# WilliamFlinchbaugh/Deep-RL-Battlespace

Measured on AMD Instinct MI355X. Metric: agent-steps/sec, higher is better.
Workload: dtype f64/i16

## Files before the change

deep-rl-battlespace_amd/csrc/bsx_kernels.hip:

```cpp

#include <array>
#include <mutex>
#include <unordered_map>

#include "bsx_config.h"
#include "bsx_args.h"
#include "bsx_state.h"
#include "bsx_rng.h"
#include "bsx_geometry.h"
#include "bsx_instinct.h"
#include "bsx_step_kernel.h"
#define BSX_INST_PER_CALL
#define BSX_INST_MULTI_TICK
#define BSX_INST_ROLLOUT
#include "bsx_step_split.h"
#define BSX_INST_SPLIT_MANY
#define BSX_INST_SPLIT
#define BSX_INST_SPLIT_CONT
#ifdef BSX_VARIANT
#define BSX_INST_KW
#else
#define BSX_INST_KW extern
#endif
#include "bsx_step_instances.h"
using namespace bsxk;

namespace {

struct ResetArgs {
    StatePtrs st; int64_t E; int n; const uint8_t* mask; const int32_t* spawn; uint64_t seed; uint64_t nonce;
    int64_t env_offset; float* obs; int observe_only;
};

__global__ __launch_bounds__(TPB) void bsx_reset_kernel(const ResetArgs p) {
    const int n = p.n, A = 2 * n, G = group_width(n), EPB = TPB / G;
    const int tid = threadIdx.x, a = tid & (G - 1), gl = tid & ~(G - 1);
    const int64_t e = int64_t(blockIdx.x) * EPB + (tid / G);
    const bool env_ok = e < p.E, valid = env_ok && a < A;
    const size_t g = valid ? size_t(e) * A + a : 0;
    __shared__ volatile int s_x[TPB], s_y[TPB], s_hp[TPB];

    EnvU er = {};
    uint32_t games = 0;
    int x = 0, y = 0, hp = 0;
    double dir = 0.0;
    bool frac = false;
    if (env_ok) {
        const uint2 dw = p.st.envd[e];
        er = unpack_env(p.st.envc[e], dw.x);
        games = dw.y;
    }
    if (valid) {
        const uint2 pw = p.st.plane[g];
        unpack_plane(pw, x, y, hp, dir);
        frac = (pw.y & PLANE_FRAC) != 0u;
        if (frac) dir = p.st.pdirf[g];
    }
    const bool doit = env_ok && !p.observe_only && (!p.mask || p.mask[e]);
    if (p.spawn) {
        if (doit) {
            const int32_t* s = p.spawn + size_t(e) * (4 + 3 * A);
            er.brx = s[0]; er.bry = s[1]; er.bbx = s[2]; er.bby = s[3];
            if (valid) { x = s[4 + 3 * a]; y = s[5 + 3 * a]; dir = double(s[6 + 3 * a]); }
        }
    } else if (!p.observe_only) {
        const int64_t genv = p.env_offset + (env_ok ? e : p.E - 1);
        const int ac = a < A ? a : A - 1;
        const SpawnDraw sd = spawn_from_words(draw4(p.seed, genv, STREAM_RESET, uint32_t(p.nonce), uint32_t(ac)), ac, n);
        const int lane0 = (tid & 63) & ~(G - 1);
        const int rbx = __shfl(sd.bx, lane0), rby = __shfl(sd.by, lane0), bbx = __shfl(sd.bx, lane0 + n), bby = __shfl(sd.by, lane0 + n);
        if (doit) {
            er.brx = rbx; er.bry = rby; er.bbx = bbx; er.bby = bby;
            if (valid) { x = sd.x; y = sd.y; dir = double(sd.dir); }
        }
    }
    if (doit) {
        er.bhp_r = er.bhp_b = 5 * n;
        er.tick = 0; er.done = 0; er.winner = BSX_WINNER_NONE;
        hp = PLANE_HP; frac = false;
        if (valid) p.st.plane[g] = pack_plane(x, y, hp, dir, false);
        if (valid && a == 0) { p.st.envc[e] = pack_envc(er); p.st.envd[e] = make_uint2(pack_envd(er), games); }
    }
    if (!p.observe_only) {
        const int lane = tid & 63;
        const int64_t wb = int64_t(blockIdx.x) * (TPB / 64) + (tid >> 6);
        const unsigned long long resetting = __ballot(doit);
        if (resetting != 0ull && wb < wave_blocks(p.E, n)) {
            uint2* const pool = p.st.bent + size_t(wb) * POOL_CAP;
            const int pc = int(p.st.bcnt[wb]);
            int wpos = 0;
            for (int base = 0; base < pc; base += 64) {
                const int w = base + lane;
                const uint2 en = pool[w < pc ? w : 0];
                const bool stay = w < pc && ((resetting >> (en.x >> ENT_OWNER_SHIFT)) & 1ull) == 0ull;
                const unsigned long long kb = __ballot(stay);
                const int ps = wpos + __popcll(kb & ((1ull << lane) - 1ull));
                if (stay) pool[ps] = en;
                wpos += __popcll(kb);
            }
            if (lane == 0) p.st.bcnt[wb] = uint32_t(wpos);
        }
    }
    s_x[tid] = x; s_y[tid] = y; s_hp[tid] = valid ? hp : 0;
    __syncthreads();
    if (valid && p.obs) {
        const int team = a < n ? 0 : 1;
        write_obs<0>(p.obs + g * size_t(3 * n + 2), n, hp > 0, x, y, dir, a,
                     team == 0 ? er.bbx : er.brx, team == 0 ? er.bby : er.bry, gl, s_x, s_y, s_hp);
    }
}

__global__ void bsx_mark_done_kernel(uint2* envd, int64_t E) {
    const int64_t e = int64_t(blockIdx.x) * blockDim.x + threadIdx.x;
    if (e < E) envd[e] = make_uint2(1u << 27, 0u);
}

struct ExportArgs { StatePtrs st; int64_t E; int n; BsxExport out; int tie_tick; };

__global__ __launch_bounds__(TPB) void bsx_export_kernel(const ExportArgs p) {
    const int A = 2 * p.n;
    const size_t EA = size_t(p.E) * A;
    const size_t g = size_t(blockIdx.x) * TPB + threadIdx.x;
    if (g >= EA) return;
    const int64_t e = int64_t(g / A);
    const int a = int(g % A);
    const uint2 pw = p.st.plane[g];
    int x, y, hp;
    double dir;
    unpack_plane(pw, x, y, hp, dir);
    if (pw.y & PLANE_FRAC) dir = p.st.pdirf[g];
    const BsxExport& o = p.out;
    if (o.px) o.px[g] = x;
    if (o.py) o.py[g] = y;
    if (o.pdir) o.pdir[g] = dir;
    if (o.php) o.php[g] = hp;
    if (o.palive) o.palive[g] = hp > 0;
    const uint2 dw = p.st.envd[e];
    const EnvU ev = unpack_env(p.st.envc[e], dw.x);
    const int ptick = ev.tick - ((ev.done && ev.winner == BSX_WINNER_TIE && ev.tick >= p.tie_tick) ? 1 : 0);
    for (int k = 0; k < K; ++k) {
        const size_t i = g * K + k;
        if (o.bl_live) o.bl_live[i] = 0;
        if (o.bl_x) o.bl_x[i] = 0;
        if (o.bl_y) o.bl_y[i] = 0;
        if (o.bl_dir) o.bl_dir[i] = 0.0;
    }
    const int G = group_width(p.n), EPB = 64 / G;
    const int64_t wb = e / EPB;
    const uint32_t me = uint32_t(int(e % EPB) * G + a);
    const uint2* const pool = p.st.bent + size_t(wb) * POOL_CAP;
    const int cnt = int(p.st.bcnt[wb]);
    for (int j2 = 0; j2 < cnt; ++j2) {
        const uint32_t w = pool[j2].x;
        const int age = bullet_age(w);
        if ((w >> ENT_OWNER_SHIFT) != me || age == int(TOMBSTONE_AGE)) continue;
        int slot = (ptick - age + 1) % K;
        if (slot < 0) slot += K;
        const size_t i = g * K + slot;
        if (o.bl_live) o.bl_live[i] = 1;
        if (o.bl_x) o.bl_x[i] = bullet_x(w);
        if (o.bl_y) o.bl_y[i] = bullet_y(w);
        if (o.bl_dir) o.bl_dir[i] = p.st.bdir[size_t(slot) * EA + g];
    }
    if (a == 0) {
        if (o.base_xy) { o.base_xy[4 * e] = ev.brx; o.base_xy[4 * e + 1] = ev.bry; o.base_xy[4 * e + 2] = ev.bbx; o.base_xy[4 * e + 3] = ev.bby; }
        if (o.bhp) { o.bhp[2 * e] = ev.bhp_r; o.bhp[2 * e + 1] = ev.bhp_b; }
        if (o.tick) o.tick[e] = ev.tick;
        if (o.env_done) o.env_done[e] = ev.done;
        if (o.winner) o.winner[e] = ev.winner;
        if (o.counters) {
            const int* c4 = p.st.cnt + 4 * e;
            o.counters[4 * e] = c4[0]; o.counters[4 * e + 1] = c4[1]; o.counters[4 * e + 2] = c4[2]; o.counters[4 * e + 3] = c4[3];
        }
    }
}

struct InstinctArgs {
    const float* obs; void* actions; const double* rnd; int64_t E; int n; int team; int out_kind; int continuous;
    uint64_t seed; uint64_t seq; const uint64_t* seq_base; int64_t env_offset;
};

__global__ __launch_bounds__(TPB) void bsx_instinct_kernel(const InstinctArgs p) {
    const int A = 2 * p.n, D = 3 * p.n + 2;
    const size_t g = size_t(blockIdx.x) * TPB + threadIdx.x;
    if (g >= size_t(p.E) * A) return;
    const int a = int(g % A);
    const int tm = a < p.n ? 0 : 1;
    if (p.team != 2 && p.team != tm) return;
    const float* o = p.obs + g * D;
    double td, ta;
    const int act = instinct_choose([&](int k) { return o[k]; }, p.n, td, ta);
    if (!p.continuous) {
        if (p.out_kind == BSX_ACT_I32) static_cast<int32_t*>(p.actions)[g] = act;
        else static_cast<float4*>(p.actions)[g] = one_hot_scores(act);
        return;
    }
    double r0, n0, n1, n2;
    if (p.rnd) { r0 = p.rnd[4 * g]; n0 = p.rnd[4 * g + 1]; n1 = p.rnd[4 * g + 2]; n2 = p.rnd[4 * g + 3]; }
    else instinct_continuous_draws(p.seed, p.seq + (p.seq_base ? *p.seq_base : 0ull), uint64_t(p.env_offset) * uint64_t(A) + g, r0, n0, n1, n2);
    double* out = static_cast<double*>(p.actions) + 3 * g;
    instinct_continuous_action(td, ta, r0, n0, n1, n2, out[0], out[1], out[2]);
}

std::mutex g_family_mu;
std::unordered_map<const void*, int> g_family;
inline void family_forget(const void* state) {
    std::lock_guard<std::mutex> lk(g_family_mu);
    g_family.erase(state);
}
inline bool family_claim(const void* state, bool cont) {
    std::lock_guard<std::mutex> lk(g_family_mu);
    int& f = g_family[state];
    if (f == 0) f = cont ? 2 : 1;
    return f == (cont ? 2 : 1);
}
inline int grid_for(int64_t E, int n) {
    const int epb = TPB / group_width(n);
    return int((E + epb - 1) / epb);
}

inline bool narrow_offsets_ok(int64_t E, int n, uint32_t flags) {
    return !(flags & BSX_F_WIDE_OFFSETS) && uint64_t(E) * uint64_t(2 * n) * 200ull <= 0xFFFFFFFFull;
}
constexpr int64_t SPLIT_MAX_GAMES = 114688, SPLIT_MANY_MAX_GAMES = 65536, SPLIT_CONT_MAX_GAMES = 81920;
constexpr int64_t SPLIT_DRAW_MAX_GAMES = 98304;
constexpr int64_t SPLIT_MANY_FORM2_FROM = 32768;
template <bool CONT, bool MULTI>
inline bool split_applies(int n, const StepArgs& a, int64_t bound) {
    if (n != 1 || (a.flags & BSX_F_ONE_WAVE)) return false;
    if (CONT) return !MULTI && bound <= SPLIT_CONT_MAX_GAMES;
    return bound <= (MULTI ? SPLIT_MANY_MAX_GAMES : SPLIT_MAX_GAMES);
}

using StepKernel = void (*)(BSX_STEP_KERNEL_PARAMS);

template <class F>
StepKernel by_team_and_offsets(int n, bool off32, F f) {
    const auto w = [&](auto N) { return off32 ? f(N, std::true_type{}) : f(N, std::false_type{}); };
    switch (n) {
        case 1: return w(std::integral_constant<int, 1>{});
        case 2: return w(std::integral_constant<int, 2>{});
        case 3: return w(std::integral_constant<int, 3>{});
        case 4: return w(std::integral_constant<int, 4>{});
        default: return w(std::integral_constant<int, 0>{});
    }
}

template <bool CONT, bool MULTI, bool ACTOR, bool LG>
int launch_for_n(const StepArgs& a, int64_t bound, void* stream) {
    const int n = a.n;
    const bool two_wave = !ACTOR && split_applies<CONT, MULTI>(n, a, bound);
    const StepKernel k = by_team_and_offsets(n, narrow_offsets_ok(a.E, n, a.flags), [&](auto N_, auto OFF32_) -> StepKernel {
        constexpr int N = decltype(N_)::value;
        constexpr bool OFF32 = decltype(OFF32_)::value;
        if constexpr (ACTOR) {
            if constexpr (N == 0) return nullptr;
            else return bsx_step_kernel<N, CONT, true, true, false, OFF32>;
        } else {
            if constexpr (N == 1 && !(CONT && MULTI)) {
                if (two_wave) {
                    if constexpr (MULTI)
                        return bound > SPLIT_MANY_FORM2_FROM ? bsx_step_split_kernel<LG, OFF32, 2>
                                                             : bsx_step_split_kernel<LG, OFF32, 1>;
                    else if constexpr (CONT)
                        return bsx_step_split_kernel<false, OFF32, 0, true, true>;
                    else
                        return bound <= SPLIT_DRAW_MAX_GAMES ? bsx_step_split_kernel<LG, OFF32, 0, false, true>
                                                             : bsx_step_split_kernel<LG, OFF32, 0>;
                }
            }
            return bsx_step_kernel<N, CONT, MULTI, false, LG, OFF32>;
        }
    });
    const StepGeometry geo = step_geometry(ACTOR ? FORM_ROLLOUT : (two_wave ? FORM_TWO_WAVE : FORM_ONE_WAVE), bound, n);
    const dim3 grid(unsigned(geo.groups));
    const dim3 block(SPB * geo.waves);
    hipLaunchKernelGGL(k, grid, block, 0, static_cast<hipStream_t>(stream),
                       bound, a.st.envc, a.st.envd, a.st.plane, a.actions, a.st.bent, a.st.bcnt, a.action_kind, a);
    return int(hipGetLastError());
}

StepArgs step_args(void* state, int64_t E, int n, int T, float* rew, uint8_t* done, uint8_t* env_done, uint8_t* winner,
                   uint8_t* env_done_t, const BsxRewards* cfg, uint32_t flags, uint64_t seed, int64_t env_offset) {
    StepArgs a{};
    a.st = state_ptrs(state, E, n);
    a.E = E; a.n = n; a.T = T;
    a.rew = rew; a.done = done; a.env_done = env_done; a.winner = winner; a.env_done_t = env_done_t;
    a.cfg = *cfg; a.flags = flags; a.seed = seed; a.env_offset = env_offset; a.tie_tick = tie_tick_const(n);
    a.scripted_team = -1;
    return a;
}

struct StepCall { int64_t first = 0, count = -1; int T = 0; int store_all = 0; uint8_t* env_done_t = nullptr; };

template <bool CONT>
int step(const StepCall& c, void* state, int64_t E, int n, const void* actions, int action_kind, const double* u, float* obs, float* rew,
         uint8_t* done, uint8_t* env_done, uint8_t* winner, const BsxRewards* cfg, uint32_t flags, uint64_t seed, int64_t env_offset,
         void* stream) {
    const int T = c.T;
    const int64_t first = c.first, count = c.count < 0 ? E - first : c.count;
    if (T < 0 || T > BSX_MAX_T || first < 0 || count <= 0 || first > E - count || (first & 255) || ((first || count != E) && T != 0))
        return BSX_E_ARG;
    if (!obs || !rew || !done || !cfg || (!actions && (T || !(flags & BSX_F_EMPTY_CALL)))) return BSX_E_ARG;
    if (const int rc = check_games(state, E, n)) return rc;
    if (!aligned(obs, 4) || !aligned(rew, 4) || (u && !aligned(u, 8))) return BSX_E_ALIGN;
    if (!CONT && action_kind == BSX_ACT_LOGITS_F32 && !aligned(actions, 16)) return BSX_E_ALIGN;
    if (!CONT && action_kind != BSX_ACT_I32 && action_kind != BSX_ACT_LOGITS_F32) return BSX_E_ARG;
    if (CONT && action_kind != BSX_ACT_F32 && action_kind != BSX_ACT_F64 && action_kind != BSX_ACT_F32X4) return BSX_E_ARG;
    if (CONT && action_kind == BSX_ACT_F32X4 && !aligned(actions, 16)) return BSX_E_ALIGN;
    if (!family_claim(state, CONT)) return BSX_E_FAMILY;
    StepArgs a = step_args(state, E, n, T, rew, done, env_done, winner, c.env_done_t, cfg, flags, seed, env_offset);
    a.actions = actions; a.action_kind = action_kind; a.u = u; a.obs = obs;
    if (!actions) { a.actions = state; a.action_kind = -1; }
    const int64_t EA = E * 2 * n;
    a.act_tb = EA * (CONT ? (action_kind == BSX_ACT_F32 ? 12 : (action_kind == BSX_ACT_F64 ? 24 : 16)) : (action_kind == BSX_ACT_I32 ? 4 : 16));
    a.u_ts = EA;
    a.obs_ts = c.store_all ? EA * (3 * n + 2) : 0; a.rew_ts = c.store_all ? EA : 0; a.done_ts = c.store_all ? EA : 0;
    if (first) {
        const int64_t fa = first * 2 * n;
        const int64_t fb = first / (64 / group_width(n));
        a.st.envc += first; a.st.envd += first; a.st.cnt += 4 * first; a.st.plane += fa; a.st.pdirf += fa;
        a.st.bcnt += fb; a.st.bent += fb * POOL_CAP; a.st.bdir += fa; a.st.bd += fa;
        if (actions) a.actions = static_cast<const char*>(actions) + fa * (a.act_tb / EA);
        if (u) a.u += fa;
        a.obs += fa * (3 * n + 2); a.rew += fa; a.done += fa;
        if (env_done) a.env_done += first;
        if (winner) a.winner += first;
        a.env_offset += first;
    }
    const bool lg = !CONT && action_kind == BSX_ACT_LOGITS_F32;
    if (T == 0) return lg ? launch_for_n<CONT, false, false, !CONT>(a, count, stream) : launch_for_n<CONT, false, false, false>(a, count, stream);
    return lg ? launch_for_n<CONT, true, false, !CONT>(a, count, stream) : launch_for_n<CONT, true, false, false>(a, count, stream);
}

template <bool CONT>
int rollout(void* state, int64_t E, int n, int T, const float* weights, int precision, int scripted_team, uint64_t scripted_seed, float* obs,
            float* scores, float* rew, uint8_t* done, uint8_t* env_done, uint8_t* winner, uint8_t* env_done_t, const BsxRewards* cfg,
            uint32_t flags, const BsxActorNoise* noise, uint64_t actor_seed, uint64_t seq, const uint64_t* seq_base, uint64_t seed,
            int64_t env_offset, void* stream, bool gauss = false, const BsxGaussianHead* head = nullptr) {
    if (T < 1 || T > BSX_MAX_T || !weights || !obs || !scores || !rew || !done || !cfg || (flags & BSX_F_EMPTY_CALL) ||
        (precision != BSX_ACTOR_F32 && precision != BSX_ACTOR_BF16X3 && precision != BSX_ACTOR_BF16X6) || scripted_team < -1 || scripted_team > 1)
        return BSX_E_ARG;
    if (gauss && (!head || !head->log_std)) return BSX_E_ARG;
    if (const int rc = check_games(state, E, n, 256, ROLLOUT_MAX_N)) return rc;
    if (!aligned(weights, 16) || !aligned(scores, 16) || !aligned(obs, 4) || !aligned(rew, 4)) return BSX_E_ALIGN;
    BsxActorNoise nz = {};
    if (noise) nz = *noise;
    if (gauss) {
        if (nz.gaussian_std > 0.f || nz.ou_scale > 0.f || nz.sample_mode != 0 || nz.u_inject || nz.logp) return BSX_E_ARG;
        if (!aligned(head->log_std, 4) || (head->logp && !aligned(head->logp, 4))) return BSX_E_ALIGN;
    }
    if (nz.ou_scale > 0.f && (!nz.ou_state || !aligned(nz.ou_state, 16))) return nz.ou_state ? BSX_E_ALIGN : BSX_E_ARG;
    if (nz.z_inject || nz.u_inject) return BSX_E_ARG;
    if (nz.sample_mode != 0 && (nz.sample_mode != 1 || !(nz.temperature > 0.f) || CONT)) return BSX_E_ARG;
    if ((nz.logp && !aligned(nz.logp, 4)) || (nz.value_weights && !aligned(nz.value_weights, 16))) return BSX_E_ALIGN;
    if (nz.value_weights && (n != 1 || !nz.value || !aligned(nz.value, 4))) return BSX_E_ARG;
    if (!family_claim(state, CONT)) return BSX_E_FAMILY;
    const int64_t EA = E * 2 * n, D = 3 * n + 2;
    StepArgs a = step_args(state, E, n, T, rew, done, env_done, winner, env_done_t, cfg, flags, seed, env_offset);
    a.action_kind = CONT ? BSX_ACT_F32X4 : BSX_ACT_LOGITS_F32;
    a.obs = obs + EA * D; a.obs_ts = EA * D; a.rew_ts = EA; a.done_ts = EA;
    a.aw = weights; a.aprec = precision; a.scripted_team = scripted_team; a.obs0 = obs; a.scores = scores; a.scores_ts = EA * 4; a.nz = nz;
    a.aseed = actor_seed; a.aseq = seq; a.aseq_base = seq_base; a.iseed = scripted_seed;
    if (gauss) a.gh = *head;
    return launch_for_n<CONT, true, true, false>(a, E, stream);
}

const std::array<double2, 361>& heading_table() {
    static const std::array<double2, 361> lut = [] {
        std::array<double2, 361> t;
        const double st = 215 * 0.1;
        for (int d = 0; d <= 360; ++d) {
            const double ang = -(double(d) * DEG2RAD);
            t[d].x = st * cos(ang);
            t[d].y = st * sin(ang);
        }
        return t;
    }();
    return lut;
}

}

extern "C" {

int bsx_abi_version(void) { return BSX_ABI_VERSION; }

int bsx_build_flags(void) { return BUILD_FLAGS; }

int bsx_stream_synchronize(void* stream) { return int(hipStreamSynchronize(static_cast<hipStream_t>(stream))); }

int bsx_host_device_pointer(void* host, void** device) {
    if (!host || !device) return BSX_E_ARG;
    return int(hipHostGetDevicePointer(device, host, 0));
}

int bsx_tie_tick(int n) { return tie_tick_const(n); }

int bsx_state_bytes(int64_t E, int n, size_t* bytes) {
    if (const int rc = check_games(bytes, E, n, 1)) return rc;
    *bytes = make_layout(E, n).total;
    return 0;
}

int bsx_state_init(void* state, int64_t E, int n, void* stream) {
    if (const int rc = check_games(state, E, n)) return rc;
    const Layout L = make_layout(E, n);
    family_forget(state);
    hipStream_t s = static_cast<hipStream_t>(stream);
    hipError_t err = hipMemsetAsync(state, 0, L.total, s);
    if (err != hipSuccess) return int(err);
    const std::array<double2, 361>& lut = heading_table();
    err = hipMemcpyAsync(static_cast<char*>(state) + L.lut, lut.data(), sizeof(double2) * lut.size(), hipMemcpyHostToDevice, s);
    if (err != hipSuccess) return int(err);
    hipLaunchKernelGGL(bsx_mark_done_kernel, dim3(unsigned((E + TPB - 1) / TPB)), dim3(TPB), 0, s,
                       reinterpret_cast<uint2*>(static_cast<char*>(state) + L.envd), E);
    return int(hipGetLastError());
}

int bsx_state_release(void* state) {
    if (!state) return BSX_E_ARG;
    family_forget(state);
    return 0;
}

int bsx_reset(void* state, int64_t E, int n, const uint8_t* reset_mask, const int32_t* spawn, uint64_t seed,
              uint64_t nonce, int64_t env_offset, float* obs, void* stream) {
    if (const int rc = check_games(state, E, n)) return rc;
    if ((spawn && !aligned(spawn, 4)) || (obs && !aligned(obs, 4))) return BSX_E_ALIGN;
    if (!reset_mask) family_forget(state);
    ResetArgs a{state_ptrs(state, E, n), E, n, reset_mask, spawn, seed, nonce, env_offset, obs, 0};
    hipLaunchKernelGGL(bsx_reset_kernel, dim3(grid_for(E, n)), dim3(TPB), 0, static_cast<hipStream_t>(stream), a);
    return int(hipGetLastError());
}

int bsx_step_discrete(void* state, int64_t E, int n, const void* actions, int action_kind, const double* u, float* obs,
                      float* rew, uint8_t* done, uint8_t* env_done, uint8_t* winner, const BsxRewards* cfg,
                      uint32_t flags, uint64_t seed, int64_t env_offset, void* stream) {
    return step<false>({}, state, E, n, actions, action_kind, u, obs, rew, done, env_done, winner, cfg, flags, seed, env_offset, stream);
}

int bsx_step_continuous(void* state, int64_t E, int n, const void* actions, int action_kind, const double* u,
                        float* obs, float* rew, uint8_t* done, uint8_t* env_done, uint8_t* winner,
                        const BsxRewards* cfg, uint32_t flags, uint64_t seed, int64_t env_offset, void* stream) {
    return step<true>({}, state, E, n, actions, action_kind, u, obs, rew, done, env_done, winner, cfg, flags, seed, env_offset, stream);
}

int bsx_step_discrete_range(void* state, int64_t E, int n, int64_t first, int64_t count, const void* actions, int action_kind, const double* u,
                            float* obs, float* rew, uint8_t* done, uint8_t* env_done, uint8_t* winner, const BsxRewards* cfg,
                            uint32_t flags, uint64_t seed, int64_t env_offset, void* stream) {
    return step<false>({first, count}, state, E, n, actions, action_kind, u, obs, rew, done, env_done, winner, cfg, flags, seed, env_offset, stream);
}

int bsx_step_continuous_range(void* state, int64_t E, int n, int64_t first, int64_t count, const void* actions, int action_kind, const double* u,
                              float* obs, float* rew, uint8_t* done, uint8_t* env_done, uint8_t* winner, const BsxRewards* cfg,
                              uint32_t flags, uint64_t seed, int64_t env_offset, void* stream) {
    return step<true>({first, count}, state, E, n, actions, action_kind, u, obs, rew, done, env_done, winner, cfg, flags, seed, env_offset, stream);
}

int bsx_step_many_discrete(void* state, int64_t E, int n, int T, const void* actions, int action_kind, const double* u,
                           float* obs, float* rew, uint8_t* done, uint8_t* env_done, uint8_t* winner, uint8_t* env_done_t, const BsxRewards* cfg,
                           uint32_t flags, int store_all, uint64_t seed, int64_t env_offset, void* stream) {
    return T < 1 ? BSX_E_ARG : step<false>({0, -1, T, store_all, env_done_t}, state, E, n, actions, action_kind, u, obs, rew, done, env_done,
                                           winner, cfg, flags, seed, env_offset, stream);
}

int bsx_step_many_continuous(void* state, int64_t E, int n, int T, const void* actions, int action_kind, const double* u,
                             float* obs, float* rew, uint8_t* done, uint8_t* env_done, uint8_t* winner, uint8_t* env_done_t, const BsxRewards* cfg,
                             uint32_t flags, int store_all, uint64_t seed, int64_t env_offset, void* stream) {
    return T < 1 ? BSX_E_ARG : step<true>({0, -1, T, store_all, env_done_t}, state, E, n, actions, action_kind, u, obs, rew, done, env_done,
                                          winner, cfg, flags, seed, env_offset, stream);
}

int bsx_rollout_discrete(void* state, int64_t E, int n, int T, const float* weights, int precision, int scripted_team, float* obs, float* scores, float* rew,
                         uint8_t* done, uint8_t* env_done, uint8_t* winner, uint8_t* env_done_t, const BsxRewards* cfg, uint32_t flags,
                         const BsxActorNoise* noise, uint64_t actor_seed, uint64_t seq, const uint64_t* seq_base, uint64_t seed,
                         int64_t env_offset, void* stream) {
    return rollout<false>(state, E, n, T, weights, precision, scripted_team, 0, obs, scores, rew, done, env_done, winner, env_done_t, cfg, flags,
                          noise, actor_seed, seq, seq_base, seed, env_offset, stream);
}

int bsx_rollout_continuous(void* state, int64_t E, int n, int T, const float* weights, int precision, int scripted_team, uint64_t scripted_seed, float* obs, float* scores, float* rew,
                           uint8_t* done, uint8_t* env_done, uint8_t* winner, uint8_t* env_done_t, const BsxRewards* cfg, uint32_t flags,
                           const BsxActorNoise* noise, uint64_t actor_seed, uint64_t seq, const uint64_t* seq_base, uint64_t seed,
                           int64_t env_offset, void* stream) {
    return rollout<true>(state, E, n, T, weights, precision, scripted_team, scripted_seed, obs, scores, rew, done, env_done, winner, env_done_t, cfg, flags,
                         noise, actor_seed, seq, seq_base, seed, env_offset, stream);
}

int bsx_rollout_continuous_gaussian(void* state, int64_t E, int n, int T, const float* weights, int precision, int scripted_team,
                                    uint64_t scripted_seed, float* obs, float* scores, float* rew,
                                    uint8_t* done, uint8_t* env_done, uint8_t* winner, uint8_t* env_done_t, const BsxRewards* cfg,
                                    uint32_t flags, const BsxActorNoise* noise, const BsxGaussianHead* head, uint64_t actor_seed,
                                    uint64_t seq, const uint64_t* seq_base, uint64_t seed, int64_t env_offset, void* stream) {
    return rollout<true>(state, E, n, T, weights, precision, scripted_team, scripted_seed, obs, scores, rew, done, env_done, winner, env_done_t, cfg, flags,
                         noise, actor_seed, seq, seq_base, seed, env_offset, stream, true, head);
}

__global__ void bsx_selftest_atan2_kernel(int R, unsigned long long* out) {
    const int W = 2 * R + 1;
    const long long total = (long long)W * W;
    unsigned long long bad = 0, seen = 0;
    for (long long i = (long long)blockIdx.x * blockDim.x + threadIdx.x; i < total; i += (long long)gridDim.x * blockDim.x) {
        const int iy = int(i / W) - R, ix = int(i % W) - R;
        const double lib = atan2(double(iy), double(ix));
        const double one = atan2_pixels(iy, ix);
        const int ys[3] = {iy, ix, -iy}, xs[3] = {ix, iy, ix};
        double three[3];
        atan2_pixels_n<3>(ys, xs, three);
        const bool ok = __double_as_longlong(one) == __double_as_longlong(lib) && __double_as_longlong(three[0]) == __double_as_longlong(lib) &&
                        __double_as_longlong(three[1]) == __double_as_longlong(atan2(double(ix), double(iy))) &&
                        __double_as_longlong(three[2]) == __double_as_longlong(atan2(double(-iy), double(ix)));
        bad += ok ? 0ull : 1ull;
        seen += 1ull;
    }
    atomicAdd(&out[0], bad); atomicAdd(&out[1], seen);
}
int bsx_selftest_atan2(int R, uint64_t* out, void* stream) {
    if (!out || R < 0 || R > 4096) return BSX_E_ARG;
    hipStream_t st = static_cast<hipStream_t>(stream);
    hipError_t err = hipMemsetAsync(out, 0, 2 * sizeof(uint64_t), st);
    if (err != hipSuccess) return int(err);
    bsx_selftest_atan2_kernel<<<1024, 256, 0, st>>>(R, reinterpret_cast<unsigned long long*>(out));
    return int(hipGetLastError());
}

int bsx_observe(void* state, int64_t E, int n, float* obs, void* stream) {
    if (!obs) return BSX_E_ARG;
    if (const int rc = check_games(state, E, n)) return rc;
    if (!aligned(obs, 4)) return BSX_E_ALIGN;
    ResetArgs a{state_ptrs(state, E, n), E, n, nullptr, nullptr, 0, 0, 0, obs, 1};
    hipLaunchKernelGGL(bsx_reset_kernel, dim3(grid_for(E, n)), dim3(TPB), 0, static_cast<hipStream_t>(stream), a);
    return int(hipGetLastError());
}

int bsx_export_state(const void* state, int64_t E, int n, const BsxExport* out, void* stream) {
    if (!out) return BSX_E_ARG;
    if (const int rc = check_games(state, E, n)) return rc;
    ExportArgs a{state_ptrs(const_cast<void*>(state), E, n), E, n, *out, bsx_tie_tick(n)};
    const size_t EA = size_t(E) * 2 * n;
    hipLaunchKernelGGL(bsx_export_kernel, dim3(unsigned((EA + TPB - 1) / TPB)), dim3(TPB), 0,
                       static_cast<hipStream_t>(stream), a);
    return int(hipGetLastError());
}

int bsx_instinct_discrete(const float* obs, void* actions, int out_kind, int64_t E, int n, int team, void* stream) {
    if (!actions || team < 0 || team > 2 || (out_kind != BSX_ACT_I32 && out_kind != BSX_ACT_LOGITS_F32)) return BSX_E_ARG;
    if (const int rc = check_games(obs, E, n, 4)) return rc;
    if (!aligned(actions, out_kind == BSX_ACT_I32 ? 4 : 16)) return BSX_E_ALIGN;
    InstinctArgs a{obs, actions, nullptr, E, n, team, out_kind, 0, 0, 0, nullptr, 0};
    const size_t EA = size_t(E) * 2 * n;
    hipLaunchKernelGGL(bsx_instinct_kernel, dim3(unsigned((EA + TPB - 1) / TPB)), dim3(TPB), 0, static_cast<hipStream_t>(stream), a);
    return int(hipGetLastError());
}

int bsx_instinct_continuous_shard(const float* obs, double* actions, const double* rnd, int64_t E, int n, int team,
                                  uint64_t seed, uint64_t seq, const uint64_t* seq_base, int64_t env_offset, void* stream) {
    if (!actions || team < 0 || team > 2 || env_offset < 0) return BSX_E_ARG;
    if (const int rc = check_games(obs, E, n, 4)) return rc;
    if (!aligned(actions, 8) || (rnd && !aligned(rnd, 8))) return BSX_E_ALIGN;
    InstinctArgs a{obs, actions, rnd, E, n, team, 0, 1, seed, seq, seq_base, env_offset};
    const size_t EA = size_t(E) * 2 * n;
    hipLaunchKernelGGL(bsx_instinct_kernel, dim3(unsigned((EA + TPB - 1) / TPB)), dim3(TPB), 0, static_cast<hipStream_t>(stream), a);
    return int(hipGetLastError());
}

int bsx_instinct_continuous(const float* obs, double* actions, const double* rnd, int64_t E, int n, int team,
                            uint64_t seed, uint64_t seq, const uint64_t* seq_base, void* stream) {
    return bsx_instinct_continuous_shard(obs, actions, rnd, E, n, team, seed, seq, seq_base, 0, stream);
}

}
```

deep-rl-battlespace_amd/csrc/bsx_step_kernel.h:

```cpp
#pragma once

namespace bsxk {

__device__ inline int argmax4(float a, float b, float c, float d) {
    int am = 0;
    float best = a;
    const float v[3] = {b, c, d};
#pragma unroll
    for (int i = 0; i < 3; ++i)
        if (!(best != best) && (v[i] > best || v[i] != v[i])) { am = i + 1; best = v[i]; }
    return am;
}

struct StepArgs {
    StatePtrs st;
    int64_t E; int n;
    const void* actions; int action_kind;
    const double* u;
    float* obs; float* rew; uint8_t* done; uint8_t* env_done; uint8_t* winner;
    uint8_t* env_done_t;
    BsxRewards cfg;
    uint32_t flags; uint64_t seed; int64_t env_offset; int tie_tick;
    int T; int64_t act_tb , u_ts, obs_ts, rew_ts, done_ts ;
    const float* aw; int aprec; int scripted_team ; const float* obs0; float* scores; int64_t scores_ts; BsxActorNoise nz; uint64_t aseed, aseq; const uint64_t* aseq_base;
    uint64_t iseed;
    BsxGaussianHead gh;
};

#define BSX_STEP_KERNEL_PARAMS                                                                                                           \
    const int64_t E_, const uint2* const envc_, const uint2* const envd_, const uint2* const plane_, const void* const act_,               \
        const uint2* const bent_, const uint32_t* const bcnt_, const int kind_, const bsxk::StepArgs p_

template <int N>
__device__ inline void write_obs(float* __restrict__ out, int n, bool alive, int x, int y, double dir, int a,
                                 int ebx, int eby, int gl, const volatile int* s_x, const volatile int* s_y,
                                 const volatile int* s_hp) {
    const int D = 3 * n + 2;
    if (!alive || (DIAG & 1u)) {
        for (int i = 0; i < D; ++i) out[i] = -1.0f;
        return;
    }
    out[0] = obs_dist(x, y, ebx, eby);
    out[1] = obs_angle(x, y, dir, ebx, eby);
    const int eb = gl + (a < n ? n : 0);
    for (int j = 0; j < n; ++j) {
        if (s_hp[eb + j] > 0) {
            const int qx = s_x[eb + j], qy = s_y[eb + j];
            out[2 + 3 * j] = 1.0f;
            out[3 + 3 * j] = obs_dist(x, y, qx, qy);
            out[4 + 3 * j] = obs_angle(x, y, dir, qx, qy);
        } else {
            out[2 + 3 * j] = -1.0f; out[3 + 3 * j] = -1.0f; out[4 + 3 * j] = -1.0f;
        }
    }
}

enum Mode : int { M_INERT = 0, M_TIE = 1, M_PHYS = 2, M_RESET = 3 };

constexpr int tie_tick_const(int n) {
    const double max_time = double(10 + n * 2);
    double t = 0.0;
    int k = 0;
    do { t += 0.1; ++k; } while (!(t >= max_time));
    return k;
}
static_assert(tie_tick_const(1) == 121 && tie_tick_const(2) == 141 && tie_tick_const(3) == 161 && tie_tick_const(4) == 181 &&
              tie_tick_const(5) == 200, "time-limit tick");
static_assert(tie_tick_const(BSX_MAX_N) < 512, "the game clock fits the 9 bits of the game record");

template <class T> __device__ inline T* elem(T* base, uint32_t i) {
    typedef typename std::conditional<std::is_const<T>::value, const char, char>::type byte_t;
    return reinterpret_cast<T*>(reinterpret_cast<byte_t*>(base) + uint32_t(i * uint32_t(sizeof(T))));
}
template <class T> __device__ inline T* elem(T* base, size_t i) { return base + i; }
__device__ inline void end_of_tick() {
    __builtin_amdgcn_fence(__ATOMIC_RELEASE, "wavefront");
    __builtin_amdgcn_wave_barrier();
    __builtin_amdgcn_fence(__ATOMIC_ACQUIRE, "wavefront");
}
template <int N, bool CONT, bool MULTI, bool ACTOR = false, bool LG = false, bool OFF32 = false>
__global__ __launch_bounds__(SPB * (ACTOR ? group_width(N > 0 ? N : 1) / 2 : WPB)) __attribute__((amdgpu_waves_per_eu((ACTOR && N > 1) ? 2 : ((!ACTOR && MULTI && N == 2) ? 4 : 1))))
void bsx_step_kernel(BSX_STEP_KERNEL_PARAMS) {
    const StepArgs& p = p_;
    const unsigned stamp_row = blockIdx.x; (void)stamp_row;
    STAMP(8);
    typedef typename std::conditional<OFF32, uint32_t, size_t>::type ix_t;
    typedef typename std::conditional<OFF32, int32_t, int64_t>::type ixs_t;
    constexpr bool NT_STATE = !MULTI && N >= 2;
    constexpr int WAVES = ACTOR ? group_width(N > 0 ? N : 1) / 2 : WPB;
    const int n = (N > 0) ? N : p.n;
    const int A = 2 * n;
    const int G = group_width(n);
    const int EPB = SPB / G;
    const int wave = (WAVES > 1) ? int(threadIdx.x >> 6) : 0;
    const int tid = (WAVES > 1) ? int(threadIdx.x & 63) : int(threadIdx.x);
    const ixs_t wblk = (WAVES > 1) ? ixs_t(blockIdx.x) * WAVES + wave : ixs_t(blockIdx.x);
    const int a = tid & (G - 1);
    const ixs_t e = wblk * EPB + (tid / G);
    const bool env_ok = e < ixs_t(E_);
    const bool valid = env_ok && a < A;
    const ix_t EA = ix_t((MULTI || ACTOR) ? E_ : p.E) * ix_t(A);
    const ixs_t ec = env_ok ? e : ixs_t(E_ - 1);
    const ix_t g = ix_t(ec) * A + (a < A ? a : A - 1);
    constexpr int MANY = -1; constexpr bool DRAW = false;
#include "bsx_step_lds.inl"

    const bool has_act = kind_ >= 0;
    struct RawIn { int ai; float4 lg; float f0, f1, f2; double c0, c1, c2, uu; };
    auto load_inputs = [&](int t, RawIn& r) {
        const void* const at = MULTI ? static_cast<const void*>(static_cast<const char*>(act_) + int64_t(t) * p.act_tb) : act_;
        const double* const ut = (MULTI && p.u) ? p.u + int64_t(t) * p.u_ts : p.u;
        if (!CONT) {
            const char* const abase = static_cast<const char*>(at);
            if constexpr (LG) r.lg = *reinterpret_cast<const float4*>(elem(abase, has_act ? g * 16 : ix_t(0)));
            else r.ai = *reinterpret_cast<const int32_t*>(elem(abase, has_act ? g * 4 : ix_t(0)));
        } else if (has_act) {
            if (kind_ == BSX_ACT_F32) {
                const float* ap = static_cast<const float*>(at) + 3 * g;
                r.f0 = ap[0]; r.f1 = ap[1]; r.f2 = ap[2];
            } else if (kind_ == BSX_ACT_F32X4) {
                const float4 v = static_cast<const float4*>(at)[g];
                r.f0 = v.x; r.f1 = v.y; r.f2 = v.z;
            } else {
                const double* ap = static_cast<const double*>(at) + 3 * g;
                r.c0 = ap[0]; r.c1 = ap[1]; r.c2 = ap[2];
            }
        }
        __builtin_amdgcn_sched_barrier(0);
        if (ut) r.uu = ut[g];
    };
    int x = 0, y = 0, hp = 0;
    uint32_t games = 0;
    double dir = 0.0;
    EnvU er = {};
    const ix_t pool0 = ix_t(wblk) * ix_t(POOL_CAP);
    uint32_t pc = 0;
    uint2 pool_first = make_uint2(0u, 0u);
    RawIn rin = {}, rin_next = {};
    struct DecIn { int act; double a0, a1, a2, uu; };
    auto decode = [&](const RawIn& r) {
        DecIn d = {-1, 0.0, 0.0, 0.0, 0.0};
        if (has_act) {
            if (!CONT) {
                if constexpr (!LG) d.act = r.ai;
                else d.act = argmax4(r.lg.x, r.lg.y, r.lg.z, r.lg.w);
            } else if (kind_ == BSX_ACT_F32 || kind_ == BSX_ACT_F32X4) {
                d.a0 = double(r.f0); d.a1 = double(r.f1); d.a2 = double(r.f2);
            } else {
                d.a0 = r.c0; d.a1 = r.c1; d.a2 = r.c2;
            }
        }
        if (p.u) d.uu = r.uu;
        return d;
    };
    DecIn din_next = {-1, 0.0, 0.0, 0.0, 0.0};
    if (MULTI && !ACTOR) { load_inputs(0, rin_next); din_next = decode(rin_next); }
    if constexpr (ACTOR) {
        constexpr int D = 3 * N + 2;
        for (int i = int(threadIdx.x); i < 2 * N * bsx_actor::SMALL / 4; i += SPB * WAVES) {
            const int ag = i / (bsx_actor::SMALL / 4), j = i - ag * (bsx_actor::SMALL / 4);
            reinterpret_cast<float4*>(s_small)[i] =
                reinterpret_cast<const float4*>(p.aw + size_t(ag) * bsx_actor::blob_floats(D) + bsx_actor::off_small(D))[j];
        }
        if constexpr (N == 1) {
            if (p.nz.value_weights)
                for (int i = int(threadIdx.x); i < 2 * bsx_actor::SMALL / 4; i += SPB * WAVES) {
                    const int ag = i / (bsx_actor::SMALL / 4), j = i - ag * (bsx_actor::SMALL / 4);
                    reinterpret_cast<float4*>(s_small + 2 * bsx_actor::SMALL)[i] =
                        reinterpret_cast<const float4*>(p.nz.value_weights + size_t(ag) * bsx_actor::blob_floats(D) + bsx_actor::off_small(D))[j];
                }
        }
        const int64_t e_first = wblk * EPB;
        const int64_t nfl = min(int64_t(SPB), (E_ - e_first) * A) * D;
        if (G == A) {
            for (int i = tid; i < SPB * D; i += SPB) s_obs[i] = i < nfl ? p.obs0[size_t(e_first) * A * D + i] : -1.0f;
        } else {
            for (int k = 0; k < D; ++k) s_obs[tid * D + k] = valid ? p.obs0[g * D + k] : -1.0f;
        }
        __builtin_amdgcn_fence(__ATOMIC_RELEASE, "workgroup");
        if (WAVES > 1) __syncthreads(); else __builtin_amdgcn_wave_barrier();
        __builtin_amdgcn_fence(__ATOMIC_ACQUIRE, "workgroup");
    }

    for (int tk = 0; tk < (MULTI ? p.T : 1); ++tk) {
    ix_t gt = g, EAt = EA;
    uint64_t seed_t = p.seed;
    int64_t env_offset_t = p.env_offset;
    constexpr int TIE_C = tie_tick_const(N > 0 ? N : 1);
    int tie_tick = (N > 0) ? TIE_C : p.tie_tick;
    if (MULTI) {
        asm volatile("" : "+v"(gt));
        asm volatile("" : "+s"(EAt));
        asm volatile("" : "+s"(seed_t));
    }
    int tid_k = tid;
    if constexpr ((ACTOR && N > 1) || (MULTI && !ACTOR && N > 0 && ((OPAQUE_MULTI_MASK >> (((LG || CONT) ? 8 : 0) + N)) & 1))) asm volatile("" : "+v"(tid_k));
    typedef const StepArgs __attribute__((address_space(4))) StepArgsK;
    static_assert(alignof(StepArgs) == 8, "kernarg offset of StepArgs");
    const char __attribute__((address_space(4)))* ka = (const char __attribute__((address_space(4)))*)__builtin_amdgcn_kernarg_segment_ptr();
    if (MULTI) asm volatile("" : "+s"(ka));
    auto& p = [&]() -> decltype(auto) { if constexpr (MULTI) return (*reinterpret_cast<StepArgsK*>(ka + 64)); else return (p_); }();
    const int tid = tid_k, lane = tid, a = tid & (G - 1);
    const int gl = tid & ~(G - 1);
    const int team = (a < n) ? 0 : 1;
    const int eb = gl + (team == 0 ? n : 0);
    const double* const u_t = (MULTI && p.u) ? p.u + int64_t(tk) * p.u_ts : p.u;
    float* const obs_t = MULTI ? p.obs + int64_t(tk) * p.obs_ts : p.obs;
    float* const rew_t = MULTI ? p.rew + int64_t(tk) * p.rew_ts : p.rew;
    uint8_t* const done_t = MULTI ? p.done + int64_t(tk) * p.done_ts : p.done;
    STAMP(0);
    if (!MULTI || tk == 0) {
        const uint2 ecw = *elem(envc_, ix_t(ec));
        const uint2 edw = *elem(envd_, ix_t(ec));
        const uint2 prw = *elem(plane_, gt);
        double dirf = 0.0;
        pool_first = *elem(bent_, pool0 + ix_t(lane));
        if (!(DIAG & 2u)) pc = __builtin_amdgcn_readfirstlane(*elem(bcnt_, ix_t(wblk)));
        if constexpr (CONT) dirf = *elem(p.st.pdirf, gt);
        if (!MULTI) load_inputs(0, rin);
        if (!MULTI) {
            asm volatile("" : "+s"(seed_t), "+s"(env_offset_t));
            if (N == 0) asm volatile("" : "+s"(tie_tick));
        }
        unpack_plane(prw, x, y, hp, dir);
        if constexpr (CONT) dir = (prw.y & PLANE_FRAC) ? dirf : dir;
        er = unpack_env(ecw, edw.x);
        games = edw.y;
    } else {
        pool_first = *elem(bent_, pool0 + ix_t(lane));
    }
    const DecIn din = MULTI ? din_next : decode(rin);
    int act = din.act;
    double a0 = din.a0, a1 = din.a1, a2 = din.a2, uu_in = din.uu;
    constexpr bool R_BULLETS = true, R_MOVE = true, R_STAGE = true, R_GEOM = true, R_OUTCOME = true, R_ST_STATE = true, R_ST_OUT = true, R_POSE_LDS = false;
    constexpr int R_RDV_COUNTS = 0, R_GEOM_LDS = 0, R_PUB = 0, R_DRAW_LDS = 0;
    auto split_rendezvous = [] {};
#include "bsx_step_phase_actor.inl"
#include "bsx_step_phase_shot.inl"
#include "bsx_step_phase_move.inl"
#include "bsx_step_phase_geometry.inl"
#include "bsx_step_phase_bullets.inl"
#include "bsx_step_phase_outcome.inl"
#include "bsx_step_phase_stores.inl"
    STAMP(7);
    if (MULTI) {
        games += uint32_t(cnt_delta.x);
        end_of_tick();
        STAMP(9);
    }
    }
}

}
```

deep-rl-battlespace_amd/csrc/bsx_step_split.h:

```cpp
#pragma once

namespace bsxk {

template <bool LG, bool OFF32, int MANY = 0, bool CONT_ = false, bool DRAW = false>
__global__ __launch_bounds__(2 * SPB)
void bsx_step_split_kernel(BSX_STEP_KERNEL_PARAMS) {
    constexpr int N = 1;
    constexpr bool CONT = CONT_, MULTI = MANY != 0, ACTOR = false;
    static_assert(!CONT || (MANY == 0 && !LG), "continuous actions: the per-call form only");
    static_assert(!DRAW || MANY == 0, "the geometry wave's draw: the per-call form only");
    const StepArgs& p = p_;
    typedef typename std::conditional<OFF32, uint32_t, size_t>::type ix_t;
    typedef typename std::conditional<OFF32, int32_t, int64_t>::type ixs_t;
    constexpr bool NT_STATE = false;
    constexpr int WAVES = 1;
    const int n = 1, A = 2, G = 2, EPB = SPB / 2;
    const int wave = 0;
    const int role_wave = int(threadIdx.x >> 6);
    const unsigned stamp_row = blockIdx.x * 2u + unsigned(role_wave); (void)stamp_row;
    STAMP(8);
    STAMP_HWID();
    const int tid = int(threadIdx.x & 63);
    const ixs_t wblk = ixs_t(blockIdx.x);
    const int a = tid & (G - 1);
    const ixs_t e = wblk * EPB + (tid / G);
    const bool env_ok = e < ixs_t(E_);
    const bool valid = env_ok && a < A;
    const ix_t EA = ix_t(MULTI ? E_ : p.E) * ix_t(A);
    const ixs_t ec = env_ok ? e : ixs_t(E_ - 1);
    const ix_t g = ix_t(ec) * A + (a < A ? a : A - 1);
#include "bsx_step_lds.inl"
    auto split_rendezvous = [] {
        asm volatile("s_waitcnt lgkmcnt(0)\n\ts_barrier" ::: "memory");
    };
    const bool has_act = kind_ >= 0;
    struct RawIn { int ai; float4 lg; double uu; };
    struct DecIn { int act; double uu; };
    auto load_inputs = [&](int t, RawIn& r) {
        const char* const abase = static_cast<const char*>(act_) + (MULTI ? int64_t(t) * p.act_tb : int64_t(0));
        if constexpr (LG) r.lg = *reinterpret_cast<const float4*>(elem(abase, has_act ? g * 16 : ix_t(0)));
        else r.ai = *reinterpret_cast<const int32_t*>(elem(abase, has_act ? g * 4 : ix_t(0)));
        __builtin_amdgcn_sched_barrier(0);
        const double* const ut = (MULTI && p.u) ? p.u + int64_t(t) * p.u_ts : p.u;
        if (ut) r.uu = ut[g];
    };
    auto decode = [&](const RawIn& r) {
        DecIn d = {-1, 0.0};
        if (has_act) d.act = LG ? argmax4(r.lg.x, r.lg.y, r.lg.z, r.lg.w) : r.ai;
        if (p.u) d.uu = r.uu;
        return d;
    };
    const ix_t pool0 = ix_t(wblk) * ix_t(POOL_CAP);
    if constexpr (MANY != 0) {
        if (role_wave == 0) {
            __builtin_amdgcn_s_setprio(1);
            constexpr bool R_BULLETS = true, R_MOVE = true, R_STAGE = true, R_GEOM = false, R_OUTCOME = true, R_POSE_LDS = false;
            constexpr bool R_ST_STATE = MANY == 2, R_ST_OUT = false;
            constexpr int R_RDV_COUNTS = MANY == 2 ? 0 : 1, R_GEOM_LDS = 0, R_PUB = MANY == 2 ? 1 : 0, R_DRAW_LDS = 0;
            s_ov[tid] = 0ull;
#include "bsx_step_split_many_body.inl"
        } else if constexpr (MANY == 2) {
            constexpr bool R_BULLETS = false, R_GEOM = true, R_ST_STATE = false, R_ST_OUT = true;
            constexpr int R_GEOM_LDS = 0, R_PUB = 0;
#include "bsx_step_split_out_body.inl"
        } else {
            constexpr bool R_BULLETS = false, R_MOVE = true, R_STAGE = false, R_GEOM = true, R_OUTCOME = true, R_POSE_LDS = false;
            constexpr bool R_ST_STATE = true, R_ST_OUT = true;
            constexpr int R_RDV_COUNTS = 2, R_GEOM_LDS = 0, R_PUB = 0, R_DRAW_LDS = 0;
#include "bsx_step_split_many_body.inl"
        }
    } else {
        constexpr int R_PUB = 0;
        const int tk = 0;
        if (role_wave == 0) {
            __builtin_amdgcn_s_setprio(1);
            constexpr bool R_BULLETS = true, R_MOVE = true, R_STAGE = true, R_GEOM = false, R_OUTCOME = true, R_ST_STATE = true, R_ST_OUT = true;
            constexpr bool R_POSE_LDS = true;
            constexpr int R_RDV_COUNTS = 0, R_GEOM_LDS = 2, R_DRAW_LDS = DRAW ? 2 : 0;
            s_ov[tid] = 0ull;
#include "bsx_step_split_body.inl"
        } else {
#include "bsx_step_split_geom_body.inl"
        }
    }
}

}
```

Baseline: 24.07 billion.

## Shrink kernel header args, read StepArgs in place, and hoist state loads

Changes the kernel parameter list to pass E as 32-bit and packs n into the kind argument, so generic-N per-call kernels read StepArgs directly from the kernarg segment at a fixed offset instead of copying it. In the per-call path, the env/plane/bullet/count state loads and the action load are issued before the tick loop so their latency overlaps setup. Continuous action loads become one unified raw-triple load with the decode deferred. This adds a hard-coded kernarg offset, and E is truncated to int, which would overflow for very large environment counts.

```diff
diff --git a/deep-rl-battlespace_amd/csrc/bsx_kernels.hip b/deep-rl-battlespace_amd/csrc/bsx_kernels.hip
--- a/deep-rl-battlespace_amd/csrc/bsx_kernels.hip
+++ b/deep-rl-battlespace_amd/csrc/bsx_kernels.hip
@@ -275,8 +275,9 @@
     const StepGeometry geo = step_geometry(ACTOR ? FORM_ROLLOUT : (two_wave ? FORM_TWO_WAVE : FORM_ONE_WAVE), bound, n);
     const dim3 grid(unsigned(geo.groups));
     const dim3 block(SPB * geo.waves);
+    const int kind_n = (!MULTI && n > 4) ? ((n << 8) | (a.action_kind & 255)) : a.action_kind;
     hipLaunchKernelGGL(k, grid, block, 0, static_cast<hipStream_t>(stream),
-                       bound, a.st.envc, a.st.envd, a.st.plane, a.actions, a.st.bent, a.st.bcnt, a.action_kind, a);
+                       int(bound), kind_n, a.st.envc, a.st.envd, a.st.plane, a.actions, a.st.bent, a.st.bcnt, a);
     return int(hipGetLastError());
 }
 
diff --git a/deep-rl-battlespace_amd/csrc/bsx_step_kernel.h b/deep-rl-battlespace_amd/csrc/bsx_step_kernel.h
--- a/deep-rl-battlespace_amd/csrc/bsx_step_kernel.h
+++ b/deep-rl-battlespace_amd/csrc/bsx_step_kernel.h
@@ -28,8 +28,10 @@
 };
 
 #define BSX_STEP_KERNEL_PARAMS                                                                                                           \
-    const int64_t E_, const uint2* const envc_, const uint2* const envd_, const uint2* const plane_, const void* const act_,               \
-        const uint2* const bent_, const uint32_t* const bcnt_, const int kind_, const bsxk::StepArgs p_
+    const int E_, const int kind_n_, const uint2* const envc_, const uint2* const envd_, const uint2* const plane_,                          \
+        const void* const act_, const uint2* const bent_, const uint32_t* const bcnt_, const bsxk::StepArgs p_
+constexpr int STEP_ARGS_KERNARG_OFFSET = 56;
+static_assert(STEP_ARGS_KERNARG_OFFSET % alignof(StepArgs) == 0, "kernarg offset of StepArgs");
 
 template <int N>
 __device__ inline void write_obs(float* __restrict__ out, int n, bool alive, int x, int y, double dir, int a,
@@ -73,6 +75,23 @@
     return reinterpret_cast<T*>(reinterpret_cast<byte_t*>(base) + uint32_t(i * uint32_t(sizeof(T))));
 }
 template <class T> __device__ inline T* elem(T* base, size_t i) { return base + i; }
+struct RawTriple { uint3 lo, hi; };
+template <class IX> __device__ inline RawTriple load_triple(const void* act, IX g, int kind, bool has_act) {
+    const char* const abase = static_cast<const char*>(act);
+    const IX stride = kind == BSX_ACT_F32 ? IX(12) : (kind == BSX_ACT_F64 ? IX(24) : IX(16));
+    const IX at = has_act ? g * stride : IX(0);
+    RawTriple r;
+    r.lo = *reinterpret_cast<const uint3*>(elem(abase, at));
+    r.hi = *reinterpret_cast<const uint3*>(elem(abase, at + (kind == BSX_ACT_F64 ? IX(12) : IX(0))));
+    return r;
+}
+__device__ inline void decode_triple(const RawTriple& r, int kind, double& a0, double& a1, double& a2) {
+    if (kind == BSX_ACT_F64) {
+        a0 = __hiloint2double(int(r.lo.y), int(r.lo.x)); a1 = __hiloint2double(int(r.hi.x), int(r.lo.z)); a2 = __hiloint2double(int(r.hi.z), int(r.hi.y));
+    } else {
+        a0 = double(__uint_as_float(r.lo.x)); a1 = double(__uint_as_float(r.lo.y)); a2 = double(__uint_as_float(r.lo.z));
+    }
+}
 __device__ inline void end_of_tick() {
     __builtin_amdgcn_fence(__ATOMIC_RELEASE, "wavefront");
     __builtin_amdgcn_wave_barrier();
@@ -81,14 +100,20 @@
 template <int N, bool CONT, bool MULTI, bool ACTOR = false, bool LG = false, bool OFF32 = false>
 __global__ __launch_bounds__(SPB * (ACTOR ? group_width(N > 0 ? N : 1) / 2 : WPB)) __attribute__((amdgpu_waves_per_eu((ACTOR && N > 1) ? 2 : ((!ACTOR && MULTI && N == 2) ? 4 : 1))))
 void bsx_step_kernel(BSX_STEP_KERNEL_PARAMS) {
-    const StepArgs& p = p_;
+    typedef const StepArgs __attribute__((address_space(4))) StepArgsK;
+    constexpr bool ARGS_IN_PLACE = N == 0 && !MULTI;
+    auto& p = [&]() -> decltype(auto) {
+        if constexpr (ARGS_IN_PLACE) return (*reinterpret_cast<StepArgsK*>((const char __attribute__((address_space(4)))*)__builtin_amdgcn_kernarg_segment_ptr() + STEP_ARGS_KERNARG_OFFSET));
+        else return (p_);
+    }();
     const unsigned stamp_row = blockIdx.x; (void)stamp_row;
     STAMP(8);
     typedef typename std::conditional<OFF32, uint32_t, size_t>::type ix_t;
     typedef typename std::conditional<OFF32, int32_t, int64_t>::type ixs_t;
     constexpr bool NT_STATE = !MULTI && N >= 2;
     constexpr int WAVES = ACTOR ? group_width(N > 0 ? N : 1) / 2 : WPB;
-    const int n = (N > 0) ? N : p.n;
+    const int kind_ = ARGS_IN_PLACE ? int(int8_t(kind_n_)) : kind_n_;
+    const int n = (N > 0) ? N : (ARGS_IN_PLACE ? (kind_n_ >> 8) : p.n);
     const int A = 2 * n;
     const int G = group_width(n);
     const int EPB = SPB / G;
@@ -99,35 +124,29 @@
     const ixs_t e = wblk * EPB + (tid / G);
     const bool env_ok = e < ixs_t(E_);
     const bool valid = env_ok && a < A;
-    const ix_t EA = ix_t((MULTI || ACTOR) ? E_ : p.E) * ix_t(A);
     const ixs_t ec = env_ok ? e : ixs_t(E_ - 1);
     const ix_t g = ix_t(ec) * A + (a < A ? a : A - 1);
     constexpr int MANY = -1; constexpr bool DRAW = false;
 #include "bsx_step_lds.inl"
 
     const bool has_act = kind_ >= 0;
-    struct RawIn { int ai; float4 lg; float f0, f1, f2; double c0, c1, c2, uu; };
-    auto load_inputs = [&](int t, RawIn& r) {
+    struct RawIn { int ai; float4 lg; RawTriple tr; double uu; };
+    auto load_action = [&](int t, RawIn& r) {
         const void* const at = MULTI ? static_cast<const void*>(static_cast<const char*>(act_) + int64_t(t) * p.act_tb) : act_;
-        const double* const ut = (MULTI && p.u) ? p.u + int64_t(t) * p.u_ts : p.u;
         if (!CONT) {
             const char* const abase = static_cast<const char*>(at);
             if constexpr (LG) r.lg = *reinterpret_cast<const float4*>(elem(abase, has_act ? g * 16 : ix_t(0)));
             else r.ai = *reinterpret_cast<const int32_t*>(elem(abase, has_act ? g * 4 : ix_t(0)));
-        } else if (has_act) {
-            if (kind_ == BSX_ACT_F32) {
-                const float* ap = static_cast<const float*>(at) + 3 * g;
-                r.f0 = ap[0]; r.f1 = ap[1]; r.f2 = ap[2];
-            } else if (kind_ == BSX_ACT_F32X4) {
-                const float4 v = static_cast<const float4*>(at)[g];
-                r.f0 = v.x; r.f1 = v.y; r.f2 = v.z;
-            } else {
-                const double* ap = static_cast<const double*>(at) + 3 * g;
-                r.c0 = ap[0]; r.c1 = ap[1]; r.c2 = ap[2];
-            }
-        }
+        } else r.tr = load_triple(at, g, kind_, has_act);
+    };
+    auto load_u = [&](int t, RawIn& r) {
+        const double* const ut = (MULTI && p.u) ? p.u + int64_t(t) * p.u_ts : p.u;
+        if (ut) r.uu = ut[g];
+    };
+    auto load_inputs = [&](int t, RawIn& r) {
+        load_action(t, r);
         __builtin_amdgcn_sched_barrier(0);
-        if (ut) r.uu = ut[g];
+        load_u(t, r);
     };
     int x = 0, y = 0, hp = 0;
     uint32_t games = 0;
@@ -144,11 +163,7 @@
             if (!CONT) {
                 if constexpr (!LG) d.act = r.ai;
                 else d.act = argmax4(r.lg.x, r.lg.y, r.lg.z, r.lg.w);
-            } else if (kind_ == BSX_ACT_F32 || kind_ == BSX_ACT_F32X4) {
-                d.a0 = double(r.f0); d.a1 = double(r.f1); d.a2 = double(r.f2);
-            } else {
-                d.a0 = r.c0; d.a1 = r.c1; d.a2 = r.c2;
-            }
+            } else decode_triple(r.tr, kind_, d.a0, d.a1, d.a2);
         }
         if (p.u) d.uu = r.uu;
         return d;
@@ -182,6 +197,21 @@
         __builtin_amdgcn_fence(__ATOMIC_ACQUIRE, "workgroup");
     }
 
+    uint2 ecw0 = make_uint2(0u, 0u), edw0 = ecw0, prw0 = ecw0;
+    uint32_t pc_raw0 = 0;
+    if constexpr (!MULTI) {
+        STAMP(0);
+        ecw0 = *elem(envc_, ix_t(ec));
+        edw0 = *elem(envd_, ix_t(ec));
+        prw0 = *elem(plane_, g);
+        pool_first = *elem(bent_, pool0 + ix_t(tid));
+        uint32_t lane0 = 0;
+        if constexpr (!OFF32) asm volatile("" : "+v"(lane0));
+        if (!(DIAG & 2u)) pc_raw0 = *elem(bcnt_, ix_t(wblk) + ix_t(lane0));
+        load_action(0, rin);
+        __builtin_amdgcn_sched_barrier(0);
+    }
+    const ix_t EA = ix_t((MULTI || ACTOR) ? E_ : p.E) * ix_t(A);
     for (int tk = 0; tk < (MULTI ? p.T : 1); ++tk) {
     ix_t gt = g, EAt = EA;
     uint64_t seed_t = p.seed;
@@ -195,11 +225,9 @@
     }
     int tid_k = tid;
     if constexpr ((ACTOR && N > 1) || (MULTI && !ACTOR && N > 0 && ((OPAQUE_MULTI_MASK >> (((LG || CONT) ? 8 : 0) + N)) & 1))) asm volatile("" : "+v"(tid_k));
-    typedef const StepArgs __attribute__((address_space(4))) StepArgsK;
-    static_assert(alignof(StepArgs) == 8, "kernarg offset of StepArgs");
     const char __attribute__((address_space(4)))* ka = (const char __attribute__((address_space(4)))*)__builtin_amdgcn_kernarg_segment_ptr();
     if (MULTI) asm volatile("" : "+s"(ka));
-    auto& p = [&]() -> decltype(auto) { if constexpr (MULTI) return (*reinterpret_cast<StepArgsK*>(ka + 64)); else return (p_); }();
+    auto& p = [&]() -> decltype(auto) { if constexpr (MULTI || ARGS_IN_PLACE) return (*reinterpret_cast<StepArgsK*>(ka + STEP_ARGS_KERNARG_OFFSET)); else return (p_); }();
     const int tid = tid_k, lane = tid, a = tid & (G - 1);
     const int gl = tid & ~(G - 1);
     const int team = (a < n) ? 0 : 1;
@@ -208,16 +236,19 @@
     float* const obs_t = MULTI ? p.obs + int64_t(tk) * p.obs_ts : p.obs;
     float* const rew_t = MULTI ? p.rew + int64_t(tk) * p.rew_ts : p.rew;
     uint8_t* const done_t = MULTI ? p.done + int64_t(tk) * p.done_ts : p.done;
-    STAMP(0);
+    if (MULTI) STAMP(0);
     if (!MULTI || tk == 0) {
-        const uint2 ecw = *elem(envc_, ix_t(ec));
-        const uint2 edw = *elem(envd_, ix_t(ec));
-        const uint2 prw = *elem(plane_, gt);
+        uint2 ecw = ecw0, edw = edw0, prw = prw0;
         double dirf = 0.0;
-        pool_first = *elem(bent_, pool0 + ix_t(lane));
-        if (!(DIAG & 2u)) pc = __builtin_amdgcn_readfirstlane(*elem(bcnt_, ix_t(wblk)));
+        if constexpr (MULTI) {
+            ecw = *elem(envc_, ix_t(ec));
+            edw = *elem(envd_, ix_t(ec));
+            prw = *elem(plane_, gt);
+            pool_first = *elem(bent_, pool0 + ix_t(lane));
+            if (!(DIAG & 2u)) pc = __builtin_amdgcn_readfirstlane(*elem(bcnt_, ix_t(wblk)));
+        } else if (!(DIAG & 2u)) pc = __builtin_amdgcn_readfirstlane(pc_raw0);
         if constexpr (CONT) dirf = *elem(p.st.pdirf, gt);
-        if (!MULTI) load_inputs(0, rin);
+        if (!MULTI) load_u(0, rin);
         if (!MULTI) {
             asm volatile("" : "+s"(seed_t), "+s"(env_offset_t));
             if (N == 0) asm volatile("" : "+s"(tie_tick));
diff --git a/deep-rl-battlespace_amd/csrc/bsx_step_split.h b/deep-rl-battlespace_amd/csrc/bsx_step_split.h
--- a/deep-rl-battlespace_amd/csrc/bsx_step_split.h
+++ b/deep-rl-battlespace_amd/csrc/bsx_step_split.h
@@ -10,6 +10,7 @@
     static_assert(!CONT || (MANY == 0 && !LG), "continuous actions: the per-call form only");
     static_assert(!DRAW || MANY == 0, "the geometry wave's draw: the per-call form only");
     const StepArgs& p = p_;
+    const int kind_ = kind_n_;
     typedef typename std::conditional<OFF32, uint32_t, size_t>::type ix_t;
     typedef typename std::conditional<OFF32, int32_t, int64_t>::type ixs_t;
     constexpr bool NT_STATE = false;
```

Result: no change. 24.31 billion, median of 6 (+1.0%).
